# sshaoshuai/PointRCNN

Measured on AMD Instinct MI355X. Metric: KITTI frames/sec, RPN inference end-to-end (16384 pts/frame, bs32 per GPU), higher is better.
Workload: dtype f32 via split-bf16x6 MFMA (every fp32 operand cut exactly into 3 bf16 pieces, 6 bf16 MFMA products per fp32 product, fp32 accumulate: fp32-grade, measured error 2.9e-7 of sum|x||w| vs 3.0e-7 for the fp32-MFMA kernel; hoisted grouped layers on the split kernel too, unhoisted grouped first layers (xyz; 1 GPU; Full RPN PointNet++ backbone (4 SA-MSG + 4 FP) + cls/reg heads, tools/cfgs/default.yaml, 16384 pts/frame, batch 32 per GPU, random-init weights, eval-mode BN; frames_per_gpu=32, npoints=16384, parallelism=frames sharded, dp1, launch=hipGraph replay, streams=20, hw_queues=4, proposal_layer=normal, clouds=uniform, group_dedup=True, roi_dedup=True

## Files before the change

### pointrcnn_amd/csrc/mlp.hip

```cpp
#include "common.h"
#include "switches.h"

#define MLP_BM 128
#define MLP_BN 64
#define MLP_BK 32
#define MLP_THREADS 256
#define MLP_ALD 36

typedef float f32x16 __attribute__((ext_vector_type(16)));

enum { MODE_PLAIN = 0, MODE_GROUP = 1, MODE_INTERP = 2 };

struct MlpParams {
    long rows;
    int K, KB, NB;
    const float* wpack;
    const float* bias;
    int Nout, relu;
    float* out;
    int ld_out, col_off, pool_ns;
    const float* in;
    int ld_in;
    const float* xyz;
    const float* new_xyz;
    const int32_t* idx;
    const float* feat;
    int ld_feat, N, M, ns, C;
    const float* known;
    const int32_t* idx3;
    const float* w3;
    const float* skip;
    int ld_known, ld_skip, n, m, C2, C1;
    int vec_a, vec_b;
    int act;
    const float* act_wx;
    const float* act_bias;
    const float* addY;
    int ldY;
    const int32_t* rows_dev;
    int rows_unit;
    const int32_t* seg_cnt;
    int seg_rows;
    int xcd_tpf;
    int wgm_cols;
    int addy_phase;
    const void* wsplit;
    int split_terms;
};

__device__ __forceinline__ long tile_of_block(const MlpParams& P, long bid) {
    if (P.xcd_tpf > 0) {
        const long xcd = bid & 7, slot = bid >> 3;
        const long k = slot / P.xcd_tpf, t = slot - k * P.xcd_tpf;
        return (k * 8 + xcd) * P.xcd_tpf + t;
    }
    if (!P.seg_cnt) return bid;
    const long nseg = P.rows / P.seg_rows, tps = P.seg_rows / 128;
    const long q = bid / nseg, sg = bid - q * nseg;
    return sg * tps + q;
}
__device__ __forceinline__ bool tile_dead(const MlpParams& P, long row0) {
    if (!P.seg_cnt) return false;
    const long s = row0 / P.seg_rows;
    return (int)(row0 - s * P.seg_rows) >= P.seg_cnt[s];
}
__device__ __forceinline__ long effective_rows(const MlpParams& P) {
    if (!P.rows_dev) return P.rows;
    const long r = (long)(*P.rows_dev) * P.rows_unit;
    return r < P.rows ? r : P.rows;
}

template <int MODE> struct RowMeta;
template <> struct RowMeta<MODE_PLAIN> { long off; bool valid; };
template <> struct RowMeta<MODE_GROUP> { long off; float dx, dy, dz; bool valid; };
template <> struct RowMeta<MODE_INTERP> { long o0, o1, o2, os; float w0, w1, w2; bool valid; };

template <int MODE> struct Raw;
template <> struct Raw<MODE_PLAIN> { float4 a; };
template <> struct Raw<MODE_GROUP> { float4 a; };
template <> struct Raw<MODE_INTERP> { float4 a, b, c; };

__host__ __device__ static inline bool aligned16(const void* p) { return (reinterpret_cast<uintptr_t>(p) & 15) == 0; }

__device__ __forceinline__ float4 ld4(const float* p) { return *reinterpret_cast<const float4*>(p); }

template <int MODE> __device__ __forceinline__ void make_meta(const MlpParams& P, long grow, RowMeta<MODE>& r);

template <> __device__ __forceinline__ void make_meta<MODE_PLAIN>(const MlpParams& P, long grow, RowMeta<MODE_PLAIN>& r) {
    r.valid = grow < P.rows;
    r.off = r.valid ? grow * (long)P.ld_in : 0;
}
template <> __device__ __forceinline__ void make_meta<MODE_GROUP>(const MlpParams& P, long grow, RowMeta<MODE_GROUP>& r) {
    r.valid = grow < P.rows;
    r.off = 0; r.dx = r.dy = r.dz = 0.f;
    if (r.valid) {
        long per_b = (long)P.M * P.ns;
        int b = (int)(grow / per_b);
        int m_ = (int)((grow - (long)b * per_b) / P.ns);
        int p = P.idx[grow];
        long pt = (long)b * P.N + p;
        r.off = pt * (long)P.ld_feat;
        float x = P.xyz[pt * 3], y = P.xyz[pt * 3 + 1], z = P.xyz[pt * 3 + 2];
        if (P.new_xyz) {
            const float* q = P.new_xyz + ((long)b * P.M + m_) * 3;
            x = x - q[0]; y = y - q[1]; z = z - q[2];
        }
        r.dx = x; r.dy = y; r.dz = z;
    }
}
template <> __device__ __forceinline__ void make_meta<MODE_INTERP>(const MlpParams& P, long grow, RowMeta<MODE_INTERP>& r) {
    r.valid = grow < P.rows;
    r.o0 = r.o1 = r.o2 = r.os = 0; r.w0 = r.w1 = r.w2 = 0.f;
    if (r.valid) {
        int b = (int)(grow / P.n);
        const int32_t* id = P.idx3 + grow * 3;
        const float* w = P.w3 + grow * 3;
        long base = (long)b * P.m;
        r.o0 = (base + id[0]) * (long)P.ld_known;
        r.o1 = (base + id[1]) * (long)P.ld_known;
        r.o2 = (base + id[2]) * (long)P.ld_known;
        r.os = grow * (long)P.ld_skip;
        r.w0 = w[0]; r.w1 = w[1]; r.w2 = w[2];
    }
}

template <int MODE> __device__ __forceinline__ void fetch(const MlpParams& P, const RowMeta<MODE>& r, int k, Raw<MODE>& v);
template <int MODE> __device__ __forceinline__ float4 finish(const MlpParams& P, const RowMeta<MODE>& r, int k, const Raw<MODE>& v);

template <> __device__ __forceinline__ void fetch<MODE_PLAIN>(const MlpParams& P, const RowMeta<MODE_PLAIN>& r, int k, Raw<MODE_PLAIN>& v) {
    v.a = make_float4(0.f, 0.f, 0.f, 0.f);
    if (!r.valid || k >= P.K) return;
    const float* s = P.in + r.off + k;
    if (P.vec_a && k + 4 <= P.K) { v.a = ld4(s); return; }
    v.a.x = s[0];
    if (k + 1 < P.K) v.a.y = s[1];
    if (k + 2 < P.K) v.a.z = s[2];
    if (k + 3 < P.K) v.a.w = s[3];
}
template <> __device__ __forceinline__ float4 finish<MODE_PLAIN>(const MlpParams&, const RowMeta<MODE_PLAIN>&, int, const Raw<MODE_PLAIN>& v) {
    return v.a;
}

__device__ __forceinline__ float group_elem(const MlpParams& P, const RowMeta<MODE_GROUP>& r, int kk) {
    if (kk < P.C) return P.feat[r.off + kk];
    if (P.act) return 0.f;
    int t = kk - P.C;
    return t == 0 ? r.dx : (t == 1 ? r.dy : (t == 2 ? r.dz : 0.f));
}
// ... 6 lines not shown
    v.a.z = group_elem(P, r, k + 2);
    v.a.w = group_elem(P, r, k + 3);
}
__device__ __forceinline__ float4 act_group4(const MlpParams& P, float4 z, int k, float dx, float dy, float dz) {
    const float4 w0 = ld4(P.act_wx + (long)k * 3), w1 = ld4(P.act_wx + (long)k * 3 + 4), w2 = ld4(P.act_wx + (long)k * 3 + 8);
    const float4 b = ld4(P.act_bias + k);
    float4 o;
    o.x = fmaxf(z.x + (w0.x * dx + w0.y * dy + w0.z * dz) + b.x, 0.f);
    o.y = fmaxf(z.y + (w0.w * dx + w1.x * dy + w1.y * dz) + b.y, 0.f);
    o.z = fmaxf(z.z + (w1.z * dx + w1.w * dy + w2.x * dz) + b.z, 0.f);
    o.w = fmaxf(z.w + (w2.y * dx + w2.z * dy + w2.w * dz) + b.w, 0.f);
    return o;
}
template <> __device__ __forceinline__ float4 finish<MODE_GROUP>(const MlpParams& P, const RowMeta<MODE_GROUP>& r, int k, const Raw<MODE_GROUP>& v) {
    if (!P.act || !r.valid || k >= P.K) return v.a;
    float4 o = act_group4(P, v.a, k, r.dx, r.dy, r.dz);
    if (k + 1 >= P.K) o.y = 0.f;
    if (k + 2 >= P.K) o.z = 0.f;
    if (k + 3 >= P.K) o.w = 0.f;
    return o;
}

__device__ __forceinline__ float interp1(float w0, float f0, float w1, float f1, float w2, float f2) {
    return __fadd_rn(__fadd_rn(__fmul_rn(w0, f0), __fmul_rn(w1, f1)), __fmul_rn(w2, f2));
}
template <> __device__ __forceinline__ void fetch<MODE_INTERP>(const MlpParams& P, const RowMeta<MODE_INTERP>& r, int k, Raw<MODE_INTERP>& v) {
    v.a = v.b = v.c = make_float4(0.f, 0.f, 0.f, 0.f);
    if (!r.valid || k >= P.K) return;
    if (k + 4 <= P.C2) {
        if (P.vec_a) {
            v.a = ld4(P.known + r.o0 + k); v.b = ld4(P.known + r.o1 + k); v.c = ld4(P.known + r.o2 + k);
        } else {
            const float *a = P.known + r.o0 + k, *b = P.known + r.o1 + k, *c = P.known + r.o2 + k;
            v.a = make_float4(a[0], a[1], a[2], a[3]);
            v.b = make_float4(b[0], b[1], b[2], b[3]);
            v.c = make_float4(c[0], c[1], c[2], c[3]);
        }
        return;
    }
    if (k >= P.C2) {
        int ks = k - P.C2;
        const float* s = P.skip + r.os + ks;
        if (P.vec_b && ks + 4 <= P.C1) { v.a = ld4(s); return; }
        if (ks < P.C1) v.a.x = s[0];
        if (ks + 1 < P.C1) v.a.y = s[1];
        if (ks + 2 < P.C1) v.a.z = s[2];
        if (ks + 3 < P.C1) v.a.w = s[3];
        return;
    }
    auto one = [&](int kk, float& a, float& b, float& c) {
        if (kk < P.C2) { a = P.known[r.o0 + kk]; b = P.known[r.o1 + kk]; c = P.known[r.o2 + kk]; }
        else if (kk - P.C2 < P.C1) { a = P.skip[r.os + kk - P.C2]; }
    };
    one(k, v.a.x, v.b.x, v.c.x);
    one(k + 1, v.a.y, v.b.y, v.c.y);
    one(k + 2, v.a.z, v.b.z, v.c.z);
    one(k + 3, v.a.w, v.b.w, v.c.w);
}
template <> __device__ __forceinline__ float4 finish<MODE_INTERP>(const MlpParams& P, const RowMeta<MODE_INTERP>& r, int k, const Raw<MODE_INTERP>& v) {
    if (k >= P.C2) return v.a;
    float4 o;
    o.x = interp1(r.w0, v.a.x, r.w1, v.b.x, r.w2, v.c.x);
    o.y = (k + 1 < P.C2) ? interp1(r.w0, v.a.y, r.w1, v.b.y, r.w2, v.c.y) : v.a.y;
    o.z = (k + 2 < P.C2) ? interp1(r.w0, v.a.z, r.w1, v.b.z, r.w2, v.c.z) : v.a.z;
    o.w = (k + 3 < P.C2) ? interp1(r.w0, v.a.w, r.w1, v.b.w, r.w2, v.c.w) : v.a.w;
    if (P.act && r.valid) {
        const float4 b = ld4(P.act_bias + k);
        o.x = fmaxf(o.x + b.x, 0.f);
        o.y = (k + 1 < P.C2) ? fmaxf(o.y + b.y, 0.f) : 0.f;
        o.z = (k + 2 < P.C2) ? fmaxf(o.z + b.z, 0.f) : 0.f;
        o.w = (k + 3 < P.C2) ? fmaxf(o.w + b.w, 0.f) : 0.f;
    }
    return o;
}

__device__ __forceinline__ float interp_gather(const MlpParams& P, long row, int n) {
    const int b = (int)(row / P.n);
    const int32_t* id = P.idx3 + row * 3;
    const float* w = P.w3 + row * 3;
    const float* y = P.addY + (long)b * P.m * P.ldY + n;
    return (w[0] * y[(long)id[0] * P.ldY] + w[1] * y[(long)id[1] * P.ldY]) + w[2] * y[(long)id[2] * P.ldY];
}

__device__ __forceinline__ void addy_stage_half(const MlpParams& P, int tid, long row0, int nb0, int hf, float* T, int ldt) {
        const int ncol0 = (nb0 + hf * 2) * 32;
        const int c = (tid & 15) * 4, n = ncol0 + c, rbase = tid >> 4;
        const bool col_ok = n < P.Nout;
        const long bfirst = row0 / P.n;
        const long next_frame_row = (bfirst + 1) * (long)P.n;
        const bool two_frames_at_most = P.n >= MLP_BM;
#pragma unroll
        for (int q = 0; q < MLP_BM / 64; q++) {
            int32_t id[4][3];
            float w[4][3];
            const float* ybase[4];
            bool ok[4];
#pragma unroll
            for (int u = 0; u < 4; u++) {
                const long g = row0 + rbase + 16 * (q * 4 + u);
                ok[u] = g < P.rows && col_ok;
                const long gg = ok[u] ? g : row0;
                const int32_t* ip = P.idx3 + gg * 3;
                const float* wp = P.w3 + gg * 3;
                id[u][0] = ip[0]; id[u][1] = ip[1]; id[u][2] = ip[2];
                w[u][0] = wp[0]; w[u][1] = wp[1]; w[u][2] = wp[2];
                const long b = two_frames_at_most ? bfirst + (gg >= next_frame_row ? 1 : 0) : gg / P.n;
                ybase[u] = P.addY + b * P.m * P.ldY + (col_ok ? n : 0);
            }
            float4 y[4][3];
#pragma unroll
            for (int u = 0; u < 4; u++)
#pragma unroll
                for (int k = 0; k < 3; k++) y[u][k] = ld4(ybase[u] + (long)id[u][k] * P.ldY);
#pragma unroll
            for (int u = 0; u < 4; u++) {
                float4 o = make_float4(0.f, 0.f, 0.f, 0.f);
                if (ok[u]) {
                    o.x = (w[u][0] * y[u][0].x + w[u][1] * y[u][1].x) + w[u][2] * y[u][2].x;
                    o.y = (w[u][0] * y[u][0].y + w[u][1] * y[u][1].y) + w[u][2] * y[u][2].y;
                    o.z = (w[u][0] * y[u][0].z + w[u][1] * y[u][1].z) + w[u][2] * y[u][2].z;
                    o.w = (w[u][0] * y[u][0].w + w[u][1] * y[u][1].w) + w[u][2] * y[u][2].w;
                }
                *reinterpret_cast<float4*>(T + (rbase + 16 * (q * 4 + u)) * ldt + c) = o;
            }
        }
    }

template <int MODE, int WNB, bool ADDY>
__device__ __forceinline__ void layer_epilogue(const MlpParams& P, f32x16 (&acc)[2][WNB], float* As0, float* Bs0, int tid, long row0,
                                               int nb0, bool n_active, bool addy_done = false) {
    const int lane = tid & 63, wave = __builtin_amdgcn_readfirstlane(tid >> 6);
    const int wm = wave >> 1, wn = wave & 1;
    const int h = lane >> 5, j = lane & 31;
    bool staged = false;
    int npass = 1;
    auto stage_half = [&](int hf, float* T, int ldt) { addy_stage_half(P, tid, row0, nb0, hf, T, ldt); };
    if (MODE == MODE_PLAIN && ADDY && P.addY && !addy_done) {
        staged = (P.Nout % 4 == 0) && (P.ldY % 4 == 0) && aligned16(P.addY);
        if (staged && Bs0) {
#pragma unroll
            for (int hf = 0; hf < WNB; hf++) stage_half(hf, hf == 0 ? As0 : Bs0, hf == 0 ? 72 : 64);
            __syncthreads();
        } else if (staged) {
            npass = WNB;
        }
    }
    if (!n_active && npass == 1) return;
    const long wrow0 = row0 + wm * 64;
#pragma unroll
    for (int pass = 0; pass < WNB; pass++) {
    if (pass >= npass) break;
    if (staged && !Bs0) {
        if (pass > 0) __syncthreads();
        stage_half(pass, As0, 72);
        __syncthreads();
    }
    if (!n_active) continue;
#pragma unroll
    for (int nn = 0; nn < WNB; nn++) {
        const int nb = nb0 + wn * WNB + nn;
        if (nb >= P.NB) continue;
        if (staged && !Bs0 && ((wn * WNB + nn) >> 1) != pass) continue;
        const int n = nb * 32 + j;
        const bool n_ok = n < P.Nout;
        const float bias = (P.bias && n_ok) ? P.bias[n] : 0.f;
        const f32x16& acc0 = acc[0][nn];
        const f32x16& acc1 = acc[1][nn];
        const bool use_addy = ADDY && P.addY && !addy_done;
        if (P.pool_ns == 0 && wrow0 + 64 <= P.rows && nb * 32 + 32 <= P.Nout && (!use_addy || staged)) {
            const int blk = wn * WNB + nn;
            const float* T = ((blk >> 1) == 0 || !Bs0) ? As0 : Bs0;
            const int ldt = ((blk >> 1) == 0 || !Bs0) ? 72 : 64, tc = (blk & 1) * 32 + j;
            float* o = P.out + (wrow0 + 4 * h) * P.ld_out + P.col_off + n;
            const long ld = P.ld_out;
#pragma unroll
            for (int r = 0; r < 16; r++) {
                const int rr = (r & 3) + 8 * (r >> 2);
                float v0 = acc0[r] + bias, v1 = acc1[r] + bias;
                if (ADDY && use_addy) {
                    v0 += T[(wm * 64 + rr + 4 * h) * ldt + tc];
                    v1 += T[(wm * 64 + 32 + rr + 4 * h) * ldt + tc];
                }
                v0 = P.relu ? fmaxf(v0, 0.f) : v0;
                v1 = P.relu ? fmaxf(v1, 0.f) : v1;
                o[rr * ld] = v0;
                o[(32 + rr) * ld] = v1;
            }
        } else if (P.pool_ns == 0) {
#pragma unroll
            for (int r = 0; r < 16; r++) {
                int rin = (r & 3) + 8 * (r >> 2) + 4 * h;
                long g0 = wrow0 + rin, g1 = wrow0 + 32 + rin;
                float v0 = acc0[r] + bias, v1 = acc1[r] + bias;
                if (ADDY && P.addY && n_ok && !addy_done) {
                    if (staged) {
                        const int blk = wn * WNB + nn;
                        const float* T = ((blk >> 1) == 0 || !Bs0) ? As0 : Bs0;
                        const int ldt = ((blk >> 1) == 0 || !Bs0) ? 72 : 64, tc = (blk & 1) * 32 + j;
                        v0 += T[(wm * 64 + rin) * ldt + tc];
                        v1 += T[(wm * 64 + 32 + rin) * ldt + tc];
                    } else {
                        if (g0 < P.rows) v0 += interp_gather(P, g0, n);
                        if (g1 < P.rows) v1 += interp_gather(P, g1, n);
                    }
                }
                if (P.relu) { v0 = fmaxf(v0, 0.f); v1 = fmaxf(v1, 0.f); }
                if (n_ok && g0 < P.rows) P.out[g0 * P.ld_out + P.col_off + n] = v0;
                if (n_ok && g1 < P.rows) P.out[g1 * P.ld_out + P.col_off + n] = v1;
            }
        } else {
            float lo0 = acc0[0], hi0 = acc0[8], lo1 = acc1[0], hi1 = acc1[8];
#pragma unroll
            for (int r = 1; r < 8; r++) {
                lo0 = fmaxf(lo0, acc0[r]); hi0 = fmaxf(hi0, acc0[8 + r]);
                lo1 = fmaxf(lo1, acc1[r]); hi1 = fmaxf(hi1, acc1[8 + r]);
            }
            lo0 = fmaxf(lo0, __shfl_xor(lo0, 32)); hi0 = fmaxf(hi0, __shfl_xor(hi0, 32));
            lo1 = fmaxf(lo1, __shfl_xor(lo1, 32)); hi1 = fmaxf(hi1, __shfl_xor(hi1, 32));
            const long groups = P.rows / P.pool_ns;
            float v[4]; long g[4]; int cnt;
            if (P.pool_ns == 16) {
                long g0 = wrow0 / 16;
                v[0] = lo0; v[1] = hi0; v[2] = lo1; v[3] = hi1; g[0] = g0; g[1] = g0 + 1; g[2] = g0 + 2; g[3] = g0 + 3; cnt = 4;
            } else if (P.pool_ns == 32) {
                long g0 = wrow0 / 32;
                v[0] = fmaxf(lo0, hi0); v[1] = fmaxf(lo1, hi1); g[0] = g0; g[1] = g0 + 1; cnt = 2;
            } else {
                v[0] = fmaxf(fmaxf(lo0, hi0), fmaxf(lo1, hi1)); g[0] = wrow0 / 64; cnt = 1;
            }
            if (h == 0 && n_ok) {
// ... 64 lines not shown
                    const float4 z = ra[u].a;
                    v.x = fmaxf(z.x + (aw0.x * dx + aw0.y * dy + aw0.z * dz) + ab.x, 0.f);
                    v.y = fmaxf(z.y + (aw0.w * dx + aw1.x * dy + aw1.y * dz) + ab.y, 0.f);
                    v.z = fmaxf(z.z + (aw1.z * dx + aw1.w * dy + aw2.x * dz) + ab.z, 0.f);
                    v.w = fmaxf(z.w + (aw2.y * dx + aw2.z * dy + aw2.w * dz) + ab.w, 0.f);
                    if (k + 1 >= P.K) v.y = 0.f;
                    if (k + 2 >= P.K) v.z = 0.f;
                    if (k + 3 >= P.K) v.w = 0.f;
                } else {
                    v = finish<MODE>(P, meta[u], k, ra[u]);
                }
            } else {
                v = finish<MODE>(P, meta[u], k, ra[u]);
            }
            *reinterpret_cast<float4*>(&As[buf][(r0 + 32 * u) * MLP_ALD + c4 * 4]) = v;
        }
#pragma unroll
        for (int u = 0; u < QN; u++) *reinterpret_cast<float4*>(&Bs[buf][(tid + 256 * u) * 4]) = rb[u];
    };

    f32x16 acc[2][WNB];
#pragma unroll
    for (int r = 0; r < 2; r++)
#pragma unroll
        for (int n = 0; n < WNB; n++) acc[r][n] = (f32x16){0};
    const bool n_active = (nb0 + wn * WNB) < P.NB;

    load_chunk(0);
    store_chunk(0, 0);
    __syncthreads();
    for (int c = 0; c < nchunks; c++) {
        const int buf = c & 1;
        if (c + 1 < nchunks) load_chunk(c + 1);
        if (n_active) {
            const int nkb = min(4, P.KB - c * 4);
            const float* a_base = &As[buf][(wm * 64 + j) * MLP_ALD + 4 * h];
            const float* b_base = &Bs[buf][wn * WNB * 1024 + lane * 4];
            for (int kbl = 0; kbl < nkb; kbl++) {
                float4 a[2], bq[WNB];
                a[0] = *reinterpret_cast<const float4*>(a_base + kbl * 8);
                a[1] = *reinterpret_cast<const float4*>(a_base + 32 * MLP_ALD + kbl * 8);
#pragma unroll
                for (int n = 0; n < WNB; n++) bq[n] = *reinterpret_cast<const float4*>(b_base + n * 1024 + kbl * 256);
#pragma unroll
                for (int r = 0; r < 2; r++)
#pragma unroll
                    for (int n = 0; n < WNB; n++) acc[r][n] = __builtin_amdgcn_mfma_f32_32x32x2f32(a[r].x, bq[n].x, acc[r][n], 0, 0, 0);
#pragma unroll
                for (int r = 0; r < 2; r++)
#pragma unroll
                    for (int n = 0; n < WNB; n++) acc[r][n] = __builtin_amdgcn_mfma_f32_32x32x2f32(a[r].y, bq[n].y, acc[r][n], 0, 0, 0);
#pragma unroll
                for (int r = 0; r < 2; r++)
#pragma unroll
                    for (int n = 0; n < WNB; n++) acc[r][n] = __builtin_amdgcn_mfma_f32_32x32x2f32(a[r].z, bq[n].z, acc[r][n], 0, 0, 0);
#pragma unroll
                for (int r = 0; r < 2; r++)
#pragma unroll
                    for (int n = 0; n < WNB; n++) acc[r][n] = __builtin_amdgcn_mfma_f32_32x32x2f32(a[r].w, bq[n].w, acc[r][n], 0, 0, 0);
            }
        }
        if (c + 1 < nchunks) store_chunk(c + 1, buf ^ 1);
        __syncthreads();
    }

    layer_epilogue<MODE, WNB, true>(P, acc, &As[0][0], &Bs[0][0], tid, row0, nb0, n_active);
}

#ifndef PRCNN_ABL
#define PRCNN_ABL 0
#endif
template <int MODE, int WNB, bool FAST, bool ADDY> struct LayerBOcc {
    static constexpr int W = ADDY ? (WNB == 1 ? 4 : 3) : (MODE == MODE_PLAIN && FAST) ? 4 : ((MODE == MODE_PLAIN || (MODE == MODE_GROUP && WNB == 1)) ? 3 : 2);
    static constexpr int RING = (MODE == MODE_PLAIN && FAST && W == 4) ? 2 : 4;
};
template <int MODE, int WNB, bool FAST, bool ADDY>
__global__ __launch_bounds__(MLP_THREADS, (LayerBOcc<MODE, WNB, FAST, ADDY>::W)) void mlp_layer_b_kernel(const MlpParams Pin) {
    MlpParams P = Pin;
    P.rows = effective_rows(Pin);
    constexpr int QN = 2 * WNB;
    long tile_id;
    int nb0;
    if (P.wgm_cols > 0) {
        const long bid = blockIdx.x, xcd = bid & 7, slot = bid >> 3;
        const long rl = slot / P.wgm_cols;
        tile_id = rl * 8 + xcd;
        nb0 = (int)(slot - rl * P.wgm_cols) * QN;
    } else {
        tile_id = tile_of_block(P, blockIdx.x);
        nb0 = blockIdx.y * QN;
    }
    if (tile_id * MLP_BM >= P.rows) return;
    if (tile_dead(P, tile_id * MLP_BM)) return;
    __shared__ __attribute__((aligned(16))) float As[2][MLP_BM * MLP_ALD];

    const int tid = threadIdx.x;
    const int lane = tid & 63, wave = __builtin_amdgcn_readfirstlane(tid >> 6);
    const int wm = wave >> 1, wn = wave & 1;
    const int h = lane >> 5, j = lane & 31;
    const long row0 = tile_id * MLP_BM;
    const int nchunks = (P.KB + 3) >> 2;

    const int c4 = tid & 7, r0 = tid >> 3;
    RowMeta<MODE> meta[4];
#pragma unroll
    for (int u = 0; u < 4; u++) {
        long grow = row0 + r0 + 32 * u;
        if (FAST && grow >= P.rows) grow = P.rows - 1;
        make_meta<MODE>(P, grow, meta[u]);
    }

    Raw<MODE> ra[4];
    const bool group_act = MODE == MODE_GROUP && P.act != 0;
    float4 aw0 = make_float4(0.f, 0.f, 0.f, 0.f), aw1 = aw0, aw2 = aw0, ab = aw0;
    auto load_chunk = [&](int c) {
        const int k = c * MLP_BK + c4 * 4;
        if constexpr (FAST) {
            if constexpr (MODE == MODE_GROUP) {
                aw0 = ld4(P.act_wx + (long)k * 3); aw1 = ld4(P.act_wx + (long)k * 3 + 4); aw2 = ld4(P.act_wx + (long)k * 3 + 8);
                ab = ld4(P.act_bias + k);
#pragma unroll
                for (int u = 0; u < 4; u++) ra[u].a = ld4(P.feat + meta[u].off + k);
            } else {
#pragma unroll
                for (int u = 0; u < 4; u++) ra[u].a = ld4(P.in + meta[u].off + k);
            }
        } else {
            if (group_act && k < P.K) {
                aw0 = ld4(P.act_wx + (long)k * 3); aw1 = ld4(P.act_wx + (long)k * 3 + 4); aw2 = ld4(P.act_wx + (long)k * 3 + 8);
                ab = ld4(P.act_bias + k);
            }
#pragma unroll
            for (int u = 0; u < 4; u++) fetch<MODE>(P, meta[u], k, ra[u]);
        }
    };
    auto store_chunk = [&](int c, int buf) {
        const int k = c * MLP_BK + c4 * 4;
#pragma unroll
        for (int u = 0; u < 4; u++) {
            float4 v;
            if constexpr (MODE == MODE_GROUP) {
                if (FAST || (group_act && meta[u].valid && k < P.K)) {
                    const float dx = meta[u].dx, dy = meta[u].dy, dz = meta[u].dz;
                    const float4 z = ra[u].a;
                    v.x = fmaxf(z.x + (aw0.x * dx + aw0.y * dy + aw0.z * dz) + ab.x, 0.f);
                    v.y = fmaxf(z.y + (aw0.w * dx + aw1.x * dy + aw1.y * dz) + ab.y, 0.f);
                    v.z = fmaxf(z.z + (aw1.z * dx + aw1.w * dy + aw2.x * dz) + ab.z, 0.f);
                    v.w = fmaxf(z.w + (aw2.y * dx + aw2.z * dy + aw2.w * dz) + ab.w, 0.f);
                    if (!FAST) {
                        if (k + 1 >= P.K) v.y = 0.f;
                        if (k + 2 >= P.K) v.z = 0.f;
                        if (k + 3 >= P.K) v.w = 0.f;
                    }
                } else {
                    v = finish<MODE>(P, meta[u], k, ra[u]);
                }
            } else if constexpr (MODE == MODE_PLAIN) {
                v = ra[u].a;
            } else {
                v = finish<MODE>(P, meta[u], k, ra[u]);
            }
            *reinterpret_cast<float4*>(&As[buf][(r0 + 32 * u) * MLP_ALD + c4 * 4]) = v;
        }
    };

    f32x16 acc[2][WNB];
#pragma unroll
    for (int r = 0; r < 2; r++)
#pragma unroll
        for (int n = 0; n < WNB; n++) acc[r][n] = (f32x16){0};
    const bool n_active = (nb0 + wn * WNB) < P.NB;

    constexpr int RING = LayerBOcc<MODE, WNB, FAST, ADDY>::RING;
    float4 bq[RING][WNB];
    const float* bptr[WNB];
#pragma unroll
    for (int n = 0; n < WNB; n++) bptr[n] = P.wpack + ((long)min(nb0 + wn * WNB + n, P.NB - 1) * P.KB) * 256 + lane * 4;
    const int kb_last = P.KB - 1;
    auto load_b = [&](int g, int slot) {
        const long off = (long)min(g, kb_last) * 256;
#pragma unroll
        for (int n = 0; n < WNB; n++) bq[slot][n] = ld4(bptr[n] + off);
    };
#pragma unroll
    for (int g = 0; g < RING; g++) load_b(g, g);

    load_chunk(0);
    bool addy_done = false;
    if constexpr (ADDY && WNB == 1) {
        const bool first = P.addY && (P.addy_phase == 2 || (P.addy_phase == 1 && ((blockIdx.x >> 8) & 1)));
        const bool stageable = (P.Nout % 4 == 0) && (P.ldY % 4 == 0) && aligned16(P.addY);
        if (first && stageable) {
            float* T = &As[0][0];
#pragma unroll
            for (int pass = 0; pass < WNB; pass++) {
                if (pass > 0) __syncthreads();
                addy_stage_half(P, tid, row0, nb0, pass, T, 72);
                __syncthreads();
#pragma unroll
                for (int nn = 0; nn < WNB; nn++) {
                    const int blk = wn * WNB + nn;
                    if ((blk >> 1) != pass) continue;
                    const int tc = (blk & 1) * 32 + j;
#pragma unroll
                    for (int r = 0; r < 16; r++) {
                        const int rin = (r & 3) + 8 * (r >> 2) + 4 * h;
                        acc[0][nn][r] = T[(wm * 64 + rin) * 72 + tc];
                        acc[1][nn][r] = T[(wm * 64 + 32 + rin) * 72 + tc];
                    }
                }
            }
            __syncthreads();
            addy_done = true;
        }
    }
    store_chunk(0, 0);
    __syncthreads();
    for (int c = 0; c < nchunks; c++) {
        const int buf = c & 1;
        if (!(PRCNN_ABL & 2)) load_chunk(min(c + 1, nchunks - 1));
        const float* a_base = &As[(PRCNN_ABL & 8) ? 0 : buf][(wm * 64 + j) * MLP_ALD + 4 * h];
#pragma unroll
        for (int kbl = 0; kbl < 4; kbl++) {
            if (n_active) {
                float4 a[2];
                a[0] = *reinterpret_cast<const float4*>(a_base + kbl * 8);
                a[1] = *reinterpret_cast<const float4*>(a_base + 32 * MLP_ALD + kbl * 8);
#pragma unroll
                for (int r = 0; r < 2; r++)
#pragma unroll
                    for (int n = 0; n < WNB; n++) acc[r][n] = __builtin_amdgcn_mfma_f32_32x32x2f32(a[r].x, bq[kbl % RING][n].x, acc[r][n], 0, 0, 0);
#pragma unroll
                for (int r = 0; r < 2; r++)
#pragma unroll
                    for (int n = 0; n < WNB; n++) acc[r][n] = __builtin_amdgcn_mfma_f32_32x32x2f32(a[r].y, bq[kbl % RING][n].y, acc[r][n], 0, 0, 0);
#pragma unroll
                for (int r = 0; r < 2; r++)
#pragma unroll
                    for (int n = 0; n < WNB; n++) acc[r][n] = __builtin_amdgcn_mfma_f32_32x32x2f32(a[r].z, bq[kbl % RING][n].z, acc[r][n], 0, 0, 0);
#pragma unroll
                for (int r = 0; r < 2; r++)
#pragma unroll
                    for (int n = 0; n < WNB; n++) acc[r][n] = __builtin_amdgcn_mfma_f32_32x32x2f32(a[r].w, bq[kbl % RING][n].w, acc[r][n], 0, 0, 0);
            }
            if (!(PRCNN_ABL & 4)) load_b(c * 4 + kbl + RING, kbl % RING);
        }
        if (!(PRCNN_ABL & 8)) {
            store_chunk(min(c + 1, nchunks - 1), buf ^ 1);
            __syncthreads();
        }
    }
    if (PRCNN_ABL & 1) {
        float sum = 0.f;
#pragma unroll
        for (int r = 0; r < 2; r++)
#pragma unroll
            for (int n = 0; n < WNB; n++)
#pragma unroll
                for (int e = 0; e < 16; e++) sum += acc[r][n][e];
        if (sum == 123.456f) P.out[tid] = sum;
        return;
    }
    layer_epilogue<MODE, WNB, ADDY>(P, acc, &As[0][0], nullptr, tid, row0, nb0, n_active, addy_done);
}

typedef __bf16 bf16x8 __attribute__((ext_vector_type(8)));
#ifndef SPL_VALU_PER_MFMA
#define SPL_VALU_PER_MFMA 5
#endif
#define SPL_LDB 80
#define SPL_PLANE (MLP_BM * SPL_LDB)

__device__ __forceinline__ void split3(float x, uint32_t& b0, uint32_t& b1, uint32_t& b2) {
    b0 = __float_as_uint(x);
    const float r1 = x - __uint_as_float(b0 & 0xFFFF0000u);
    b1 = __float_as_uint(r1);
    const float r2 = r1 - __uint_as_float(b1 & 0xFFFF0000u);
    b2 = __float_as_uint(r2);
}
__device__ __forceinline__ uint32_t bf16_pair(uint32_t lo, uint32_t hi) { return __builtin_amdgcn_perm(hi, lo, 0x07060302u); }

__global__ void pack_weight_split_kernel(const float* __restrict__ w, int Nout, int K, int KS, int NB, int chain, uint4* __restrict__ img) {
    const long e = (long)blockIdx.x * blockDim.x + threadIdx.x;
    if (e >= (long)NB * KS * 64) return;
    const int lane = (int)(e & 63);
    long blk = e >> 6;
    const int ks = (int)(blk % KS), nb = (int)(blk / KS);
    const int n = nb * 32 + (lane & 31), hh = lane >> 5;
    uint32_t b[3][8];
#pragma unroll
    for (int i = 0; i < 8; i++) {
        const int k = chain ? ks * 16 + 8 * (i >> 2) + 4 * hh + (i & 3) : ks * 16 + 8 * hh + i;
        const float v = (n < Nout && k < K) ? w[(long)n * K + k] : 0.f;
        split3(v, b[0][i], b[1][i], b[2][i]);
    }
    if (chain) blk = (long)ks * NB + nb;
#pragma unroll
    for (int p = 0; p < 3; p++)
        img[(blk * 3 + p) * 64 + lane] = make_uint4(bf16_pair(b[p][0], b[p][1]), bf16_pair(b[p][2], b[p][3]),
                                                    bf16_pair(b[p][4], b[p][5]), bf16_pair(b[p][6], b[p][7]));
}

template <int NR>
__device__ __forceinline__ bool wave_has_nonfinite(const f32x16 (&acc)[NR]) {
    float chk = 0.f;
#pragma unroll
    for (int r = 0; r < NR; r++)
#pragma unroll
        for (int e = 0; e < 16; e++) chk = __builtin_fmaf(acc[r][e], 0.f, chk);
    return __builtin_amdgcn_ballot_w64(chk != chk) != 0;
}

template <int MODE, int WNB>
__device__ __forceinline__ void split_redo_f32(const MlpParams& P, f32x16 (&acc)[2][WNB], long row0, int wm, int wn, int nb0, int lane) {
    const int h = lane >> 5, j = lane & 31;
    const float* ar[2];
    const float* bp[WNB];
    float gd[2][3] = {{0.f, 0.f, 0.f}, {0.f, 0.f, 0.f}};
#pragma unroll
    for (int r = 0; r < 2; r++) {
        long g = row0 + wm * 64 + r * 32 + j;
        if (g >= P.rows) g = P.rows - 1;
        if constexpr (MODE == MODE_GROUP) {
            RowMeta<MODE_GROUP> gm;
            make_meta<MODE_GROUP>(P, g, gm);
            ar[r] = P.feat + gm.off + 4 * h;
            gd[r][0] = gm.dx; gd[r][1] = gm.dy; gd[r][2] = gm.dz;
        } else {
            ar[r] = P.in + g * P.ld_in + 4 * h;
        }
    }
#pragma unroll
    for (int n = 0; n < WNB; n++) bp[n] = P.wpack + ((long)min(nb0 + wn * WNB + n, P.NB - 1) * P.KB) * 256 + lane * 4;
#pragma unroll
    for (int r = 0; r < 2; r++)
#pragma unroll
        for (int n = 0; n < WNB; n++) acc[r][n] = (f32x16){0};
    for (int kb = 0; kb < P.KB; kb++) {
        float4 a[2], b[WNB];
#pragma unroll
        for (int r = 0; r < 2; r++) {
            a[r] = ld4(ar[r] + kb * 8);
            if constexpr (MODE == MODE_GROUP) a[r] = act_group4(P, a[r], kb * 8 + 4 * h, gd[r][0], gd[r][1], gd[r][2]);
        }
#pragma unroll
        for (int n = 0; n < WNB; n++) b[n] = ld4(bp[n] + (long)kb * 256);
#pragma unroll
        for (int r = 0; r < 2; r++)
#pragma unroll
            for (int n = 0; n < WNB; n++) acc[r][n] = __builtin_amdgcn_mfma_f32_32x32x2f32(a[r].x, b[n].x, acc[r][n], 0, 0, 0);
#pragma unroll
        for (int r = 0; r < 2; r++)
#pragma unroll
            for (int n = 0; n < WNB; n++) acc[r][n] = __builtin_amdgcn_mfma_f32_32x32x2f32(a[r].y, b[n].y, acc[r][n], 0, 0, 0);
#pragma unroll
        for (int r = 0; r < 2; r++)
#pragma unroll
            for (int n = 0; n < WNB; n++) acc[r][n] = __builtin_amdgcn_mfma_f32_32x32x2f32(a[r].z, b[n].z, acc[r][n], 0, 0, 0);
#pragma unroll
        for (int r = 0; r < 2; r++)
#pragma unroll
            for (int n = 0; n < WNB; n++) acc[r][n] = __builtin_amdgcn_mfma_f32_32x32x2f32(a[r].w, b[n].w, acc[r][n], 0, 0, 0);
    }
}

template <int MODE, int WNB, int TERMS, bool ADDY>
__device__ __forceinline__ void layer_s_tile(const MlpParams& P, const long bx, const int by, const int tid, unsigned char* __restrict__ Ls) {
    constexpr int QN = 2 * WNB;
    constexpr int NP = TERMS == 6 ? 3 : 2;
    long tile_id;
    int nb0;
    if (P.wgm_cols > 0) {
        const long bid = bx, xcd = bid & 7, slot = bid >> 3;
        const long rl = slot / P.wgm_cols;
        tile_id = rl * 8 + xcd;
        nb0 = (int)(slot - rl * P.wgm_cols) * QN;
    } else {
        tile_id = tile_of_block(P, bx);
        nb0 = by * QN;
    }
    if (tile_id * MLP_BM >= P.rows) return;
    if (tile_dead(P, tile_id * MLP_BM)) return;

    const int lane = tid & 63, wave = __builtin_amdgcn_readfirstlane(tid >> 6);
    const int wm = wave >> 1, wn = wave & 1;
    const int h = lane >> 5, j = lane & 31;
    const long row0 = tile_id * MLP_BM;
    const int nchunks = P.K / MLP_BK, KS = P.K / 16;

    static_assert(MODE == MODE_PLAIN || (MODE == MODE_GROUP && !ADDY), "split layer kernel: plain rows or the hoisted grouped form");
    const int c4 = tid & 7, r0 = tid >> 3;
    const float* arow[4];
    float gdx[4], gdy[4], gdz[4];
#pragma unroll
    for (int u = 0; u < 4; u++) {
        long grow = row0 + r0 + 32 * u;
        if (grow >= P.rows) grow = P.rows - 1;
        if constexpr (MODE == MODE_GROUP) {
            RowMeta<MODE_GROUP> gm;
            make_meta<MODE_GROUP>(P, grow, gm);
            arow[u] = P.feat + gm.off + c4 * 4;
            gdx[u] = gm.dx; gdy[u] = gm.dy; gdz[u] = gm.dz;
        } else {
            arow[u] = P.in + grow * P.ld_in + c4 * 4;
            gdx[u] = gdy[u] = gdz[u] = 0.f;
        }
    }
    float4 raA[4], raB[4];
    auto load_chunk = [&](int c, float4 (&ra)[4]) {
#pragma unroll
        for (int u = 0; u < 4; u++) ra[u] = ld4(arow[u] + c * MLP_BK);
    };
    auto store_chunk = [&](int buf, const float4 (&ra)[4], int c) {
#pragma unroll
        for (int u = 0; u < 4; u++) {
            float4 v = ra[u];
            if constexpr (MODE == MODE_GROUP) v = act_group4(P, v, c * MLP_BK + c4 * 4, gdx[u], gdy[u], gdz[u]);
            uint32_t b[3][4];
            split3(v.x, b[0][0], b[1][0], b[2][0]);
            split3(v.y, b[0][1], b[1][1], b[2][1]);
            split3(v.z, b[0][2], b[1][2], b[2][2]);
            split3(v.w, b[0][3], b[1][3], b[2][3]);
#pragma unroll
            for (int p = 0; p < NP; p++)
                *reinterpret_cast<uint2*>(Ls + (buf * 3 + p) * SPL_PLANE + (r0 + 32 * u) * SPL_LDB + c4 * 8) =
                    make_uint2(bf16_pair(b[p][0], b[p][1]), bf16_pair(b[p][2], b[p][3]));
        }
    };

    f32x16 acc[2][WNB];
#pragma unroll
    for (int r = 0; r < 2; r++)
#pragma unroll
        for (int n = 0; n < WNB; n++) acc[r][n] = (f32x16){0};
    const bool n_active = (nb0 + wn * WNB) < P.NB;

    uint4 bq[2][WNB][NP];
    const uint4* bptr[WNB];
#pragma unroll
    for (int n = 0; n < WNB; n++) bptr[n] = reinterpret_cast<const uint4*>(P.wsplit) + ((long)min(nb0 + wn * WNB + n, P.NB - 1) * KS) * 192 + lane;
    auto load_b = [&](int g, int slot) {
        const long off = (long)min(g, KS - 1) * 192;
#pragma unroll
        for (int n = 0; n < WNB; n++)
#pragma unroll
            for (int p = 0; p < NP; p++) bq[slot][n][p] = bptr[n][off + p * 64];
    };
    bf16x8 a0[2][NP], a1[2][NP];
    auto read_a = [&](int buf, int st, bf16x8 (&a)[2][NP]) {
        const unsigned char* a_base = Ls + buf * 3 * SPL_PLANE + (wm * 64 + j) * SPL_LDB + h * 16 + st * 32;
#pragma unroll
        for (int r = 0; r < 2; r++)
#pragma unroll
            for (int p = 0; p < NP; p++)
                a[r][p] = __builtin_bit_cast(bf16x8, *reinterpret_cast<const uint4*>(a_base + p * SPL_PLANE + r * 32 * SPL_LDB));
    };
#define SPL_TERM(A, SL, PA, PB)                                                                                                   \
    _Pragma("unroll") for (int r = 0; r < 2; r++) _Pragma("unroll") for (int n = 0; n < WNB; n++)                                  \
        acc[r][n] = __builtin_amdgcn_mfma_f32_32x32x16_bf16(A[r][PA], __builtin_bit_cast(bf16x8, bq[SL][n][PB]), acc[r][n], 0, 0, 0)
#define SPL_STEP(A, SL)                                                                                 \
    do {                                                                                                                          \
        if constexpr (TERMS == 6) { SPL_TERM(A, SL, 0, 2); SPL_TERM(A, SL, 2, 0); SPL_TERM(A, SL, 1, 1); }                         \
        SPL_TERM(A, SL, 0, 1); SPL_TERM(A, SL, 1, 0); SPL_TERM(A, SL, 0, 0);                                                       \
    } while (0)
    constexpr int NM = 2 * WNB * TERMS;
    load_b(0, 0);
    load_b(1, 1);
    load_chunk(0, raA);
    load_chunk(min(1, nchunks - 1), raB);
    bool addy_done = false;
    if constexpr (ADDY) {
        const bool stageable = P.addY && P.addy_phase != 0 && (P.Nout % 4 == 0) && (P.ldY % 4 == 0) && aligned16(P.addY);
        if (stageable) {
            float* T = reinterpret_cast<float*>(Ls);
#pragma unroll
            for (int pass = 0; pass < WNB; pass++) {
                if (pass > 0) __syncthreads();
                addy_stage_half(P, tid, row0, nb0, pass, T, 72);
                __syncthreads();
#pragma unroll
                for (int nn = 0; nn < WNB; nn++) {
                    const int blk = wn * WNB + nn;
                    if ((blk >> 1) != pass) continue;
                    const int tc = (blk & 1) * 32 + j;
#pragma unroll
                    for (int r = 0; r < 16; r++) {
                        const int rin = (r & 3) + 8 * (r >> 2) + 4 * h;
                        acc[0][nn][r] = T[(wm * 64 + rin) * 72 + tc];
                        acc[1][nn][r] = T[(wm * 64 + 32 + rin) * 72 + tc];
                    }
                }
            }
            __syncthreads();
            addy_done = true;
        }
    }
    store_chunk(0, raA, 0);
    __syncthreads();
    read_a(0, 0, a0);
    if (PRCNN_ABL & 256) read_a(0, 1, a1);
    auto chunk_body = [&](int c, const float4 (&ra_split)[4], float4 (&ra_load)[4]) {
        const int buf = c & 1;
        if (!(PRCNN_ABL & 64)) load_chunk(min(c + 2, nchunks - 1), ra_load);
        if (!(PRCNN_ABL & 256)) read_a(buf, 1, a1);
        if (!(PRCNN_ABL & 128)) SPL_STEP(a0, 0);
        if (!(PRCNN_ABL & 32)) load_b(c * 2 + 2, 0);
#pragma unroll
        for (int q = 0; q < 2 * NP; q++) {
            __builtin_amdgcn_sched_group_barrier(0x008, 1, 0);
            __builtin_amdgcn_sched_group_barrier(0x100, 1, 0);
        }
#pragma unroll
        for (int q = 0; q < 4 + WNB * NP; q++) {
            __builtin_amdgcn_sched_group_barrier(0x008, 1, 0);
            __builtin_amdgcn_sched_group_barrier(0x020, 1, 0);
        }
        __builtin_amdgcn_sched_barrier(0);
        if (!(PRCNN_ABL & 64)) store_chunk(buf ^ 1, ra_split, min(c + 1, nchunks - 1));
        if (!(PRCNN_ABL & 128)) SPL_STEP(a1, 1);
        if (!(PRCNN_ABL & 32)) load_b(c * 2 + 3, 1);
#pragma unroll
        for (int q = 0; q < NM; q++) {
            __builtin_amdgcn_sched_group_barrier(0x008, 1, 0);
            __builtin_amdgcn_sched_group_barrier(0x002, SPL_VALU_PER_MFMA, 0);
            if (q % 2 == 1 && q / 2 < 4 * NP) __builtin_amdgcn_sched_group_barrier(0x200, 1, 0);
        }
        __builtin_amdgcn_sched_barrier(0);
        if (!(PRCNN_ABL & 256)) {
            __syncthreads();
            read_a(buf ^ 1, 0, a0);
        }
    };
    for (int c = 0; c < nchunks; c += 2) {
        chunk_body(c, raB, raA);
        if (c + 1 < nchunks) chunk_body(c + 1, raA, raB);
    }
#undef SPL_STEP
#undef SPL_TERM
    if (PRCNN_ABL & (16 | 128)) {
        float sum = 0.f;
#pragma unroll
        for (int r = 0; r < 2; r++)
#pragma unroll
            for (int n = 0; n < WNB; n++)
#pragma unroll
                for (int e = 0; e < 16; e++) sum += acc[r][n][e];
        if (PRCNN_ABL & 128) {
#pragma unroll
            for (int r = 0; r < 2; r++)
#pragma unroll
                for (int p = 0; p < NP; p++) sum += (float)a0[r][p][0] + (float)a1[r][p][3] + __uint_as_float(bq[0][0][p].x) + __uint_as_float(bq[1][WNB - 1][p].w);
        }
        if (sum == 123.456f) P.out[tid] = sum;
        if (PRCNN_ABL & 16) return;
    }
    if (!(PRCNN_ABL & (16 | 128))) {
        bool bad = wave_has_nonfinite<2 * WNB>(reinterpret_cast<const f32x16 (&)[2 * WNB]>(acc));
        if (ADDY && addy_done) bad = __syncthreads_or(bad) != 0;
        if (bad && n_active) split_redo_f32<MODE, WNB>(P, acc, row0, wm, wn, nb0, lane);
        if (bad) addy_done = false;
    }
    layer_epilogue<MODE, WNB, ADDY>(P, acc, reinterpret_cast<float*>(Ls), nullptr, tid, row0, nb0, n_active, addy_done);
}

template <int MODE, int WNB, int TERMS, bool ADDY, bool LOOP>
__global__ __launch_bounds__(MLP_THREADS, 2) void mlp_layer_s_kernel(const MlpParams Pin) {
    MlpParams P = Pin;
    P.rows = effective_rows(Pin);
    __shared__ __attribute__((aligned(16))) unsigned char Ls[2 * 3 * SPL_PLANE];
    if constexpr (LOOP) {
        const long nbid = ((P.rows + MLP_BM - 1) / MLP_BM + 7) / 8 * 8 * P.wgm_cols;
        for (long bid = blockIdx.x; bid < nbid; bid += gridDim.x) {
            int tid;
            asm volatile("v_mov_b32 %0, %1" : "=v"(tid) : "v"(threadIdx.x));
            layer_s_tile<MODE, WNB, TERMS, ADDY>(P, bid, 0, tid, Ls);
            __syncthreads();
        }
    } else {
        layer_s_tile<MODE, WNB, TERMS, ADDY>(P, blockIdx.x, blockIdx.y, threadIdx.x, Ls);
    }
}

struct ChainParams {
    MlpParams a;
    const float* wpack1; const float* bias1; int KB1, N1, relu1;
    const float* wpack2; const float* bias2; int KB2, N2, relu2;
    int nlayers;
    int stack_split;
    const void* wsplit1;
};

#define CH_DPP_FMAX(v, ctrl) asm volatile("s_nop 1\n\tv_max_f32_dpp %0, %0, %0 " ctrl : "+v"(v))
#define CH_DPP_FMAX4(v, ctrl)                                                                                   \
    asm volatile("s_nop 1\n\tv_max_f32_dpp %0, %0, %0 " ctrl "\n\tv_max_f32_dpp %1, %1, %1 " ctrl               \
                 "\n\tv_max_f32_dpp %2, %2, %2 " ctrl "\n\tv_max_f32_dpp %3, %3, %3 " ctrl                       \
                 : "+v"(v[0]), "+v"(v[1]), "+v"(v[2]), "+v"(v[3]))

__device__ __forceinline__ float4 ldw(const float* __restrict__ wpack, int KB, int ob, int kb, int lane) {
    return ld4(wpack + (((long)ob * KB + kb) * 64 + lane) * 4);
}

template <int NB>
__device__ __forceinline__ void bias_act(f32x16 (&acc)[NB], const float* __restrict__ bias, int relu, int h) {
#pragma unroll
    for (int ob = 0; ob < NB; ob++)
#pragma unroll
        for (int q = 0; q < 4; q++) {
            float4 b = bias ? ld4(bias + ob * 32 + 8 * q + 4 * h) : make_float4(0.f, 0.f, 0.f, 0.f);
            float v0 = acc[ob][4 * q + 0] + b.x, v1 = acc[ob][4 * q + 1] + b.y;
            float v2 = acc[ob][4 * q + 2] + b.z, v3 = acc[ob][4 * q + 3] + b.w;
            if (relu) { v0 = fmaxf(v0, 0.f); v1 = fmaxf(v1, 0.f); v2 = fmaxf(v2, 0.f); v3 = fmaxf(v3, 0.f); }
            acc[ob][4 * q + 0] = v0; acc[ob][4 * q + 1] = v1; acc[ob][4 * q + 2] = v2; acc[ob][4 * q + 3] = v3;
        }
}

#define CH_WAVES 4
#define CH_STAGE_TILES 16
template <int NB> struct ChStage { static constexpr int G = CH_STAGE_TILES / NB; static constexpr int TPW = (G * NB + CH_WAVES - 1) / CH_WAVES; };

template <int NB>
__device__ __forceinline__ void stage_load(const float* __restrict__ wpack, int KB, int st, int wave, int lane, float4 (&r)[4]) {
    constexpr int G = ChStage<NB>::G;
#pragma unroll
    for (int u = 0; u < ChStage<NB>::TPW; u++) {
        int tt = wave + CH_WAVES * u, kbl = tt / NB, ob = tt - kbl * NB, kb = st * G + kbl;
        r[u] = (tt < G * NB && kb < KB) ? ldw(wpack, KB, ob, kb, lane) : make_float4(0.f, 0.f, 0.f, 0.f);
    }
}
template <int NB>
__device__ __forceinline__ void stage_store(float* ws, int wave, int lane, const float4 (&r)[4]) {
#pragma unroll
    for (int u = 0; u < ChStage<NB>::TPW; u++) {
        int tt = wave + CH_WAVES * u;
        if (tt < ChStage<NB>::G * NB) *reinterpret_cast<float4*>(ws + (tt * 64 + lane) * 4) = r[u];
    }
}
__device__ __forceinline__ float4 lds_w(const float* ws, int tile, int lane) {
    return *reinterpret_cast<const float4*>(ws + (tile * 64 + lane) * 4);
}

template <int NBI, int NBO>
__device__ __forceinline__ void chain_layer(const f32x16 (&in)[NBI], f32x16 (&out)[NBO], const float* __restrict__ wpack,
                                            int KB, float (*Ws)[CH_STAGE_TILES * 256], int wave, int lane) {
    constexpr int G = ChStage<NBO>::G;
    constexpr int NST = (NBI * 4 + G - 1) / G;
// ... 1505 lines not shown
```

Measured before the change: 15080 frames/s.

## Stage interpolation indices in LDS and order addend tiles by frame per XCD

Interpolation-addend layers now load each tile's three neighbour indices and weights once per row into shared memory. The staging passes read them from there instead of re-reading them from global memory in every half-pass and epilogue. Tile-to-block mapping also changes when the frame size is a multiple of 128 and the frame count a multiple of 8: each XCD then processes whole frames' tiles contiguously, so the gathered addY rows for a frame stay in that XCD's L2. The cost is extra LDS, an added barrier before staging, and changed block scheduling order.

```diff
diff --git a/pointrcnn_amd/csrc/mlp.hip b/pointrcnn_amd/csrc/mlp.hip
--- a/pointrcnn_amd/csrc/mlp.hip
+++ b/pointrcnn_amd/csrc/mlp.hip
@@ -1,5 +1,6 @@
 #include "common.h"
 #include "switches.h"
+#include "tile_order.h"
 
 #define MLP_BM 128
 #define MLP_BN 64
@@ -64,6 +65,11 @@
     const long s = row0 / P.seg_rows;
     return (int)(row0 - s * P.seg_rows) >= P.seg_cnt[s];
 }
+template <bool ADDY>
+__device__ __forceinline__ int addy_frame_rows(const MlpParams& P) {
+    if constexpr (!ADDY) return 0;
+    return (P.addY && !P.rows_dev && !P.seg_cnt) ? P.n : 0;
+}
 __device__ __forceinline__ long effective_rows(const MlpParams& P) {
     if (!P.rows_dev) return P.rows;
     const long r = (long)(*P.rows_dev) * P.rows_unit;
@@ -236,7 +242,20 @@
     return (w[0] * y[(long)id[0] * P.ldY] + w[1] * y[(long)id[1] * P.ldY]) + w[2] * y[(long)id[2] * P.ldY];
 }
 
-__device__ __forceinline__ void addy_stage_half(const MlpParams& P, int tid, long row0, int nb0, int hf, float* T, int ldt) {
+#define ADDY_IDX_WORDS (2 * MLP_BM * 3)
+__device__ __forceinline__ void addy_load_index(const MlpParams& P, int tid, long row0, uint32_t (&v)[3]) {
+    const int r = tid & (MLP_BM - 1);
+    const long g = row0 + r;
+    const long gg = g < P.rows ? g : row0;
+    const uint32_t* src = tid < MLP_BM ? reinterpret_cast<const uint32_t*>(P.idx3) : reinterpret_cast<const uint32_t*>(P.w3);
+    v[0] = src[gg * 3]; v[1] = src[gg * 3 + 1]; v[2] = src[gg * 3 + 2];
+}
+__device__ __forceinline__ void addy_store_index(int tid, const uint32_t (&v)[3], uint32_t* S) {
+    S[tid * 3] = v[0]; S[tid * 3 + 1] = v[1]; S[tid * 3 + 2] = v[2];
+}
+
+template <bool SIDX>
+__device__ __forceinline__ void addy_stage_half(const MlpParams& P, int tid, long row0, int nb0, int hf, float* T, int ldt, const uint32_t* S) {
         const int ncol0 = (nb0 + hf * 2) * 32;
         const int c = (tid & 15) * 4, n = ncol0 + c, rbase = tid >> 4;
         const bool col_ok = n < P.Nout;
@@ -251,13 +270,20 @@
             bool ok[4];
 #pragma unroll
             for (int u = 0; u < 4; u++) {
-                const long g = row0 + rbase + 16 * (q * 4 + u);
+                const int rl = rbase + 16 * (q * 4 + u);
+                const long g = row0 + rl;
                 ok[u] = g < P.rows && col_ok;
                 const long gg = ok[u] ? g : row0;
-                const int32_t* ip = P.idx3 + gg * 3;
-                const float* wp = P.w3 + gg * 3;
-                id[u][0] = ip[0]; id[u][1] = ip[1]; id[u][2] = ip[2];
-                w[u][0] = wp[0]; w[u][1] = wp[1]; w[u][2] = wp[2];
+                if constexpr (SIDX) {
+                    const uint32_t* sp = S + (ok[u] ? rl : 0) * 3;
+                    id[u][0] = (int32_t)sp[0]; id[u][1] = (int32_t)sp[1]; id[u][2] = (int32_t)sp[2];
+                    w[u][0] = __uint_as_float(sp[MLP_BM * 3]); w[u][1] = __uint_as_float(sp[MLP_BM * 3 + 1]); w[u][2] = __uint_as_float(sp[MLP_BM * 3 + 2]);
+                } else {
+                    const int32_t* ip = P.idx3 + gg * 3;
+                    const float* wp = P.w3 + gg * 3;
+                    id[u][0] = ip[0]; id[u][1] = ip[1]; id[u][2] = ip[2];
+                    w[u][0] = wp[0]; w[u][1] = wp[1]; w[u][2] = wp[2];
+                }
                 const long b = two_frames_at_most ? bfirst + (gg >= next_frame_row ? 1 : 0) : gg / P.n;
                 ybase[u] = P.addY + b * P.m * P.ldY + (col_ok ? n : 0);
             }
@@ -280,17 +306,25 @@
         }
     }
 
-template <int MODE, int WNB, bool ADDY>
+template <int MODE, int WNB, bool ADDY, bool SIDX = false>
 __device__ __forceinline__ void layer_epilogue(const MlpParams& P, f32x16 (&acc)[2][WNB], float* As0, float* Bs0, int tid, long row0,
-                                               int nb0, bool n_active, bool addy_done = false) {
+                                               int nb0, bool n_active, bool addy_done = false, uint32_t* S = nullptr) {
     const int lane = tid & 63, wave = __builtin_amdgcn_readfirstlane(tid >> 6);
     const int wm = wave >> 1, wn = wave & 1;
     const int h = lane >> 5, j = lane & 31;
     bool staged = false;
     int npass = 1;
-    auto stage_half = [&](int hf, float* T, int ldt) { addy_stage_half(P, tid, row0, nb0, hf, T, ldt); };
+    auto stage_half = [&](int hf, float* T, int ldt) { addy_stage_half<SIDX>(P, tid, row0, nb0, hf, T, ldt, S); };
     if (MODE == MODE_PLAIN && ADDY && P.addY && !addy_done) {
         staged = (P.Nout % 4 == 0) && (P.ldY % 4 == 0) && aligned16(P.addY);
+        if constexpr (SIDX) {
+            if (staged) {
+                uint32_t iw[3];
+                addy_load_index(P, tid, row0, iw);
+                addy_store_index(tid, iw, S);
+                __syncthreads();
+            }
+        }
         if (staged && Bs0) {
 #pragma unroll
             for (int hf = 0; hf < WNB; hf++) stage_half(hf, hf == 0 ? As0 : Bs0, hf == 0 ? 72 : 64);
@@ -299,7 +333,7 @@
             npass = WNB;
         }
     }
-    if (!n_active && npass == 1) return;
+    if (!n_active && !(staged && !Bs0)) return;
     const long wrow0 = row0 + wm * 64;
 #pragma unroll
     for (int pass = 0; pass < WNB; pass++) {
@@ -530,10 +564,9 @@
     long tile_id;
     int nb0;
     if (P.wgm_cols > 0) {
-        const long bid = blockIdx.x, xcd = bid & 7, slot = bid >> 3;
-        const long rl = slot / P.wgm_cols;
-        tile_id = rl * 8 + xcd;
-        nb0 = (int)(slot - rl * P.wgm_cols) * QN;
+        const TileOfBlock tb = tile_order(blockIdx.x, P.rows, addy_frame_rows<ADDY>(P), P.wgm_cols);
+        tile_id = tb.tile_id;
+        nb0 = tb.col * QN;
     } else {
         tile_id = tile_of_block(P, blockIdx.x);
         nb0 = blockIdx.y * QN;
@@ -541,6 +574,7 @@
     if (tile_id * MLP_BM >= P.rows) return;
     if (tile_dead(P, tile_id * MLP_BM)) return;
     __shared__ __attribute__((aligned(16))) float As[2][MLP_BM * MLP_ALD];
+    __shared__ uint32_t Ix[ADDY_IDX_WORDS];
 
     const int tid = threadIdx.x;
     const int lane = tid & 63, wave = __builtin_amdgcn_readfirstlane(tid >> 6);
@@ -630,20 +664,24 @@
 #pragma unroll
         for (int n = 0; n < WNB; n++) bq[slot][n] = ld4(bptr[n] + off);
     };
+    uint32_t iw[3] = {0u, 0u, 0u};
+    if constexpr (ADDY && WNB == 1) addy_load_index(P, tid, row0, iw);
 #pragma unroll
     for (int g = 0; g < RING; g++) load_b(g, g);
 
     load_chunk(0);
+    if constexpr (ADDY && WNB == 1) addy_store_index(tid, iw, Ix);
     bool addy_done = false;
     if constexpr (ADDY && WNB == 1) {
         const bool first = P.addY && (P.addy_phase == 2 || (P.addy_phase == 1 && ((blockIdx.x >> 8) & 1)));
         const bool stageable = (P.Nout % 4 == 0) && (P.ldY % 4 == 0) && aligned16(P.addY);
         if (first && stageable) {
             float* T = &As[0][0];
+            __syncthreads();
 #pragma unroll
             for (int pass = 0; pass < WNB; pass++) {
                 if (pass > 0) __syncthreads();
-                addy_stage_half(P, tid, row0, nb0, pass, T, 72);
+                addy_stage_half<true>(P, tid, row0, nb0, pass, T, 72, Ix);
                 __syncthreads();
 #pragma unroll
                 for (int nn = 0; nn < WNB; nn++) {
@@ -709,7 +747,9 @@
         if (sum == 123.456f) P.out[tid] = sum;
         return;
     }
-    layer_epilogue<MODE, WNB, ADDY>(P, acc, &As[0][0], nullptr, tid, row0, nb0, n_active, addy_done);
+    uint32_t* Sx = nullptr;
+    if constexpr (ADDY) Sx = Ix;
+    layer_epilogue<MODE, WNB, ADDY, ADDY>(P, acc, &As[0][0], nullptr, tid, row0, nb0, n_active, addy_done, Sx);
 }
 
 typedef __bf16 bf16x8 __attribute__((ext_vector_type(8)));
@@ -819,10 +859,9 @@
     long tile_id;
     int nb0;
     if (P.wgm_cols > 0) {
-        const long bid = bx, xcd = bid & 7, slot = bid >> 3;
-        const long rl = slot / P.wgm_cols;
-        tile_id = rl * 8 + xcd;
-        nb0 = (int)(slot - rl * P.wgm_cols) * QN;
+        const TileOfBlock tb = tile_order(bx, P.rows, addy_frame_rows<ADDY>(P), P.wgm_cols);
+        tile_id = tb.tile_id;
+        nb0 = tb.col * QN;
     } else {
         tile_id = tile_of_block(P, bx);
         nb0 = by * QN;
@@ -912,19 +951,25 @@
         SPL_TERM(A, SL, 0, 1); SPL_TERM(A, SL, 1, 0); SPL_TERM(A, SL, 0, 0);                                                       \
     } while (0)
     constexpr int NM = 2 * WNB * TERMS;
+    uint32_t iw[3] = {0u, 0u, 0u};
+    uint32_t* const Sx = reinterpret_cast<uint32_t*>(Ls) + MLP_BM * 72;
+    static_assert((MLP_BM * 72 + ADDY_IDX_WORDS) * 4 <= 2 * 3 * SPL_PLANE && MLP_BM * 72 * 4 >= 3 * SPL_PLANE, "addend tile + index words: in the operand LDS, past buffer 0");
+    if constexpr (ADDY) addy_load_index(P, tid, row0, iw);
     load_b(0, 0);
     load_b(1, 1);
     load_chunk(0, raA);
     load_chunk(min(1, nchunks - 1), raB);
+    if constexpr (ADDY) addy_store_index(tid, iw, Sx);
     bool addy_done = false;
     if constexpr (ADDY) {
         const bool stageable = P.addY && P.addy_phase != 0 && (P.Nout % 4 == 0) && (P.ldY % 4 == 0) && aligned16(P.addY);
         if (stageable) {
             float* T = reinterpret_cast<float*>(Ls);
+            __syncthreads();
 #pragma unroll
             for (int pass = 0; pass < WNB; pass++) {
                 if (pass > 0) __syncthreads();
-                addy_stage_half(P, tid, row0, nb0, pass, T, 72);
+                addy_stage_half<true>(P, tid, row0, nb0, pass, T, 72, Sx);
                 __syncthreads();
 #pragma unroll
                 for (int nn = 0; nn < WNB; nn++) {
@@ -1008,7 +1053,7 @@
         if (bad && n_active) split_redo_f32<MODE, WNB>(P, acc, row0, wm, wn, nb0, lane);
         if (bad) addy_done = false;
     }
-    layer_epilogue<MODE, WNB, ADDY>(P, acc, reinterpret_cast<float*>(Ls), nullptr, tid, row0, nb0, n_active, addy_done);
+    layer_epilogue<MODE, WNB, ADDY, ADDY>(P, acc, reinterpret_cast<float*>(Ls), nullptr, tid, row0, nb0, n_active, addy_done, Sx);
 }
 
 template <int MODE, int WNB, int TERMS, bool ADDY, bool LOOP>
diff --git a/pointrcnn_amd/csrc/tile_order.h b/pointrcnn_amd/csrc/tile_order.h
--- /dev/null
+++ b/pointrcnn_amd/csrc/tile_order.h
@@ -0,0 +1,30 @@
+#pragma once
+#include <hip/hip_runtime.h>
+
+struct TileOfBlock {
+    long tile_id;
+    int col;
+};
+
+__host__ __device__ inline bool tile_order_by_frame(long rows, int frame_n) {
+    if (frame_n <= 0 || (frame_n & 127) != 0) return false;
+    const long frames = rows / frame_n;
+    return frames * frame_n == rows && frames > 0 && (frames & 7) == 0;
+}
+
+__host__ __device__ inline TileOfBlock tile_order(long bid, long rows, int frame_n, int cols) {
+    const long xcd = bid & 7, slot = bid >> 3;
+    TileOfBlock r;
+    if (tile_order_by_frame(rows, frame_n)) {
+        const long tpf = frame_n >> 7, per = tpf * cols;
+        const long k = slot / per, t = slot - k * per;
+        const long tr = t / cols;
+        r.tile_id = (k * 8 + xcd) * tpf + tr;
+        r.col = (int)(t - tr * cols);
+    } else {
+        const long rl = slot / cols;
+        r.tile_id = rl * 8 + xcd;
+        r.col = (int)(slot - rl * cols);
+    }
+    return r;
+}
```

Measured after the change: 15250 frames/s, median of 4. About the same (+1.1%).
